# TencentARC/BlobCtrl

Hardware: AMD Instinct MI355X
Metric: 512x512_50step_blobctrl_edits_per_sec (higher is better)
Workload: dtype fp16

## Files before the change

__graft_entry__.py:

```python
import os
import subprocess
import sys

REPO = os.path.dirname(os.path.abspath(__file__))
CSRC = os.path.join(REPO, "blobctrl_amd", "csrc")
LIB = os.path.join(REPO, "blobctrl_amd", "libblobctrl_hip.so")
HEADERS = [os.path.join(REPO, "include", h) for h in ("blobctrl_hip.h", "blobctrl_vae.h")]
SOURCES = ["gemm.hip", "gemm_fast.hip", "conv_halo.hip", "conv_wreg.hip", "gemm_wreg.hip", "gemm256.hip", "norm.hip", "attention.hip", "rowchain.hip", "rowchain_midx.hip", "elementwise.hip", "blobviz.hip", "freeu.hip", "vae_tile.hip", "capi.hip", "plan.hip"]


def _stale():
    if not os.path.exists(LIB):
        return True
    t = os.path.getmtime(LIB)
    deps = [os.path.join(CSRC, f) for f in os.listdir(CSRC)] + HEADERS
    return any(os.path.getmtime(d) > t for d in deps)


def _compile_one(args):
    src, obj, flags = args
    subprocess.check_call([os.environ.get("HIPCC", "/opt/rocm/bin/hipcc")] + flags + ["-c", src, "-o", obj])
    return obj


# ... 60 lines not shown
```

blobctrl_amd/_lib.py:

```python
import ctypes as C
import os

_HERE = os.path.dirname(os.path.abspath(__file__))
LIB_PATH = os.environ.get("BLOBCTRL_HIP_LIB") or os.path.join(_HERE, "libblobctrl_hip.so")

A_DENSE, A_CONV3X3 = 0, 1
ACT_NONE, ACT_GELU, ACT_GEGLU, ACT_SILU, ACT_QUICK_GELU = 0, 1, 2, 3, 4
OUT_F16, OUT_F16_T, OUT_F32 = 0, 1, 2
TILE_NAMES = ["auto", "256x128", "128x128_s3", "128x128_s2", "256x64_s2", "256x64_s3", "128x64", "64x64", "halo128x160", "wreg128x160",
              "gw64x128", "gw64x256", "gw64x320", "g256x256"]
TILE_HALO = 8
TILE_WREG = 9
TILE_GW64x128, TILE_GW64x256, TILE_GW64x320 = 10, 11, 12
TILE_G256 = 13
GW_TILES = {TILE_GW64x128: 2, TILE_GW64x256: 4, TILE_GW64x320: 5}


class BcGemm(C.Structure):
    _fields_ = [
        ("A", C.c_void_p), ("A2", C.c_void_p), ("a_mode", C.c_int),
        ("M", C.c_int), ("N", C.c_int), ("K", C.c_int),
        ("lda", C.c_int), ("lda2", C.c_int), ("C1", C.c_int), ("Cin", C.c_int),
        ("Hin", C.c_int), ("Win", C.c_int), ("Hv", C.c_int), ("Wv", C.c_int),
        ("Hout", C.c_int), ("Wout", C.c_int), ("stride", C.c_int), ("conv_nopad_lo", C.c_int),
# ... 132 lines not shown
    "bc_event_create_sync": (C.c_int, [C.POINTER(C.c_void_p)]),
    "bc_stream_wait_event": (C.c_int, [C.c_void_p, C.c_void_p]),
    "bc_event_record": (C.c_int, [C.c_void_p, C.c_void_p]),
    "bc_event_elapsed_ms": (C.c_int, [C.c_void_p, C.c_void_p, C.POINTER(C.c_float)]),
    "bc_event_destroy": (C.c_int, [C.c_void_p]),
}

EXPORTED_SYMBOLS = tuple(_SIGNATURES.keys())

VAE_SIGNATURES = {
    "bc_vae_tile_blend": (C.c_int, [C.c_void_p, C.c_void_p, C.c_void_p, C.c_void_p, C.c_void_p, C.c_int, C.c_int, C.c_int, C.c_int, C.c_int,
                                    C.c_int, C.c_int, C.c_int, C.c_int, C.c_int, C.c_int, C.c_int, C.c_int, C.c_int, C.c_void_p]),
}
VAE_TILE_DECODE, VAE_TILE_ENCODE = 0, 1

OPS = {"bc_gemm": 0, "bc_gn_stats": 1, "bc_gn_finalize": 2, "bc_gn_apply_fused": 3, "bc_gn_apply": 4, "bc_layernorm": 5,
       "bc_attention": 6, "bc_attention_causal": 7, "bc_assemble_input": 8, "bc_timestep_embedding": 9,
       "bc_timestep_embedding_table": 10, "bc_cfg_scheduler_step": 11, "bc_embed_tokens": 12, "bc_softmax_rows": 13,
       "bc_patchify": 14, "bc_add_cls_pos": 15, "bc_silu": 16, "bc_nchw_to_nhwc_f16": 17, "bc_nhwc_to_nchw": 18,
       "bc_gaussian_sample": 19, "bc_rowchain": 22, "bc_assemble_input_im2col": 23, "bc_memset_zero": 24,
       "bc_rowchain_midx": 25, "bc_rowchain_pack_kv": 26, "bc_rowchain_sum": 27, "bc_ctx_fold": 28, "bc_dup_halves": 29,
       "bc_cfg_scheduler_step_noise": 30, "bc_cfg_scheduler_step3": 31,
       "bc_assemble_input_scaled": 32, "bc_assemble_input_im2col_scaled": 33, "bc_scheduler_step_single": 34,
       "bc_timestep_embedding_table_cond": 35, "bc_timestep_embedding_cond": 36, "bc_freeu": 37}
OP_SIGNAL, OP_WAIT = 20, 21
CHAIN_IN, CHAIN_MID, CHAIN_OUT, CHAIN_OUT_FF, CHAIN_OUT_TAIL, CHAIN_MIDX, CHAIN_OUT_FFP = 0, 1, 2, 3, 4, 5, 6
GN_TOT_WORDS = 6
_KIND = {C.c_void_p: "p", C.c_int: "i", C.c_float: "f", C.c_longlong: "l", C.c_char_p: "p"}


def op_signature(name):
    args = _SIGNATURES[name][1][:-1]
    return "".join("p" if (a not in _KIND) else _KIND[a] for a in args)


class BcPlanBuffer(C.Structure):
    _fields_ = [("name", C.c_char_p), ("address", C.c_void_p), ("bytes", C.c_longlong), ("host_data", C.c_void_p)]

_lib = None


class BlobCtrlHipError(RuntimeError):
    pass


def load():
    global _lib
    if _lib is not None:
        return _lib
    if not os.path.exists(LIB_PATH):
        raise BlobCtrlHipError(
            f"{LIB_PATH} not found: build it with `python -c 'import __graft_entry__ as g; g.build()'` "
            "(hipcc --offload-arch=gfx950).  blobctrl_amd has no CPU fallback.")
    try:
        import torch
    except ImportError:
        pass
    try:
        lib = C.CDLL(LIB_PATH)
    except OSError as e:
        raise BlobCtrlHipError(f"failed to load {LIB_PATH}: {e}") from e
    for name, (res, args) in list(_SIGNATURES.items()) + list(VAE_SIGNATURES.items()):
        fn = getattr(lib, name)
        fn.restype = res
        fn.argtypes = args
    if lib.bc_sizeof_gemm() != C.sizeof(BcGemm):
        raise BlobCtrlHipError(f"BcGemm layout mismatch: C {lib.bc_sizeof_gemm()} vs ctypes {C.sizeof(BcGemm)}")
    _lib = lib
    return lib


def check(rc, what=""):
    if rc != 0:
        msg = load().bc_last_error()
        raise BlobCtrlHipError(f"{what} failed (rc={rc}): {msg.decode() if msg else ''}")
```

blobctrl_amd/csrc/elementwise.hip:

```cpp
#include "bc_common.h"
#include "bc_splat.h"

namespace {

__global__ void splat_kernel(const SplatParams prm, int h, int w, double* __restrict__ out) {
    const int n = blockIdx.y;
    const int idx = blockIdx.x * blockDim.x + threadIdx.x;
    if (idx >= h * w) return;
    const int gy = idx / w, gx = idx - gy * w;
    const double s = bc_splat_score(prm.v + n * 8, gx, gy, h, w);
    double* o = out + (size_t)n * 2 * h * w;
    o[idx] = (1.0 - s);
    o[(size_t)h * w + idx] = s;
}

__device__ __forceinline__ float input_divisor(const float* __restrict__ coef, const int* __restrict__ step_idx, int nsteps) {
    const int step = *step_idx;
    return (step >= 0 && step < nsteps) ? coef[(size_t)step * 16 + 14] : 1.f;
}

template <bool SCALED>
__global__ void assemble_kernel(const float* __restrict__ latents, int Blat, const float* __restrict__ img_lat,
                                const float* __restrict__ score, const float* __restrict__ feat, int Bimg, int F, int Bout,
                                int h, int w, int Cpad, int dup_score, const float* __restrict__ coef,
// ... 109 lines not shown
template <bool SINGLE, bool NOISE, bool THIRD, bool GUARD>
__device__ __forceinline__ void cfg_step_body(const float* __restrict__ eps, float* __restrict__ latents, const float* __restrict__ coef,
                                              const int* __restrict__ step_idx, float* __restrict__ hist, float guidance, int B, int h,
                                              int w, const float* __restrict__ noise, int nsteps, float* __restrict__ eps_out) {
    const int n = B * 4 * h * w;
    const int i = blockIdx.x * blockDim.x + threadIdx.x;
    const int step = *step_idx;
    if (i >= n) return;
    if (GUARD && (step < 0 || step >= nsteps)) return;
    const float* cf = coef + (size_t)step * 16;
    const int xx = i % w;
    const int yy = (i / w) % h;
    const int c = (i / (w * h)) % 4;
    const int b = i / (4 * w * h);
    const size_t pu = (((size_t)b * h + yy) * (2 * w) + (w + xx)) * 4 + c;
    float e;
    if (SINGLE) {
        e = eps[pu];
    } else {
        const size_t pc = (((size_t)(B + b) * h + yy) * (2 * w) + (w + xx)) * 4 + c;
        const float eu = eps[pu], ec = eps[pc];
        const float gscale = guidance >= 0.f ? guidance : cf[11];
        e = eu + gscale * (ec - eu);
    }
    if (eps_out) eps_out[i] = e;
    const float x = latents[i];
    float* m0 = hist, *m1 = hist + n, *last = hist + 2 * (size_t)n;
    const float x0 = x * cf[0] - e * cf[1];
    float xc = x;
    const float pm0 = m0[i], pm1 = m1[i];
    if (cf[2] != 0.f) xc = cf[3] * last[i] + cf[4] * pm0 + cf[5] * pm1 + cf[6] * x0;
    float xn = cf[7] * xc + cf[8] * x0 + cf[9] * pm0 + cf[10] * e;
    m1[i] = pm0;
    m0[i] = x0;
    last[i] = xc;
    if (NOISE) xn = xn + cf[12] * noise[(size_t)step * n + i];
    if (THIRD) xn = xn + cf[13] * pm1;
    latents[i] = xn;
}

template <bool NOISE, bool THIRD, bool GUARD>
__global__ void cfg_step_kernel(const float* __restrict__ eps, float* __restrict__ latents, const float* __restrict__ coef,
                                const int* __restrict__ step_idx, float* __restrict__ hist, float guidance, int B, int h, int w,
                                const float* __restrict__ noise, int nsteps, float* __restrict__ eps_out) {
    cfg_step_body<false, NOISE, THIRD, GUARD>(eps, latents, coef, step_idx, hist, guidance, B, h, w, noise, nsteps, eps_out);
}

template <bool NOISE, bool THIRD>
__global__ void step_single_kernel(const float* __restrict__ eps, float* __restrict__ latents, const float* __restrict__ coef,
                                   const int* __restrict__ step_idx, float* __restrict__ hist, int B, int h, int w,
                                   const float* __restrict__ noise, int nsteps, float* __restrict__ eps_out) {
    cfg_step_body<true, NOISE, THIRD, true>(eps, latents, coef, step_idx, hist, 0.f, B, h, w, noise, nsteps, eps_out);
}
// ... 350 lines not shown
```

blobctrl_amd/csrc/plan.hip:

```cpp
#include <stdio.h>
#include <string.h>
#include <map>
#include <string>
#include <vector>
#include "bc_common.h"
#include "plan_format.h"

void bc_gemm_set_probe(hipEvent_t e);
bool bc_gemm_probe_hit();

using namespace bcplan;

namespace {

struct EventSet {
    std::vector<hipEvent_t> ev;
    explicit EventSet(size_t n) : ev(n, nullptr) {}
    ~EventSet() { for (auto e : ev) if (e) (void)hipEventDestroy(e); }
    hipEvent_t& operator[](size_t i) { return ev[i]; }
};

struct Seg {
    std::string name;
    std::vector<Rec> recs;
// ... 94 lines not shown
            return bc_assemble_input_scaled(CP(float, 0), I(1), CP(float, 2), CP(float, 3), CP(float, 4), I(5), I(6), I(7), I(8), I(9), I(10),
                                            I(11), CP(float, 12), CP(int, 13), I(14), MP(bc_half, 15), s);
        case BC_OP_ASSEMBLE_IM2COL_SCALED:
            return bc_assemble_input_im2col_scaled(CP(float, 0), I(1), CP(float, 2), CP(float, 3), I(4), I(5), I(6), I(7), I(8), CP(float, 9),
                                                   CP(int, 10), I(11), MP(bc_half, 12), s);
        case BC_OP_SCHEDULER_STEP_SINGLE:
            return bc_scheduler_step_single(CP(float, 0), MP(float, 1), CP(float, 2), MP(int, 3), MP(float, 4), I(5), I(6), I(7), CP(float, 8),
                                            I(9), I(10), MP(float, 11), I(12), s);
        case BC_OP_TIMESTEP_EMBEDDING_TABLE_COND:
            return bc_timestep_embedding_table_cond(CP(float, 0), I(1), I(2), I(3), CP(float, 4), MP(bc_half, 5), s);
        case BC_OP_TIMESTEP_EMBEDDING_COND:
            return bc_timestep_embedding_cond(CP(float, 0), CP(int, 1), F(2), I(3), I(4), CP(float, 5), MP(bc_half, 6), s);
        case BC_OP_FREEU:
            return bc_freeu(CP(bc_half, 0), I(1), CP(bc_half, 2), I(3), I(4), I(5), CP(float, 6), I(7), CP(float, 8), MP(bc_half, 9),
                            MP(bc_half, 10), MP(unsigned long long, 11), MP(unsigned long long, 12), s);
        case BC_OP_ROWCHAIN:
            return bc_rowchain(I(0), I(1), I(2), I(3), CP(bc_half, 4), CP(float, 5), CP(unsigned long long, 6), CP(float, 7), CP(float, 8), I(9),
                               F(10), CP(bc_half, 11), CP(bc_half, 12), CP(bc_half, 13), I(14), I(15), I(16), CP(bc_half, 17), CP(float, 18),
                               MP(bc_half, 19), MP(bc_half, 20), MP(bc_half, 21), I(22), MP(unsigned long long, 23), F(24), F(25),
                               CP(float, 26), CP(int, 27), I(28), MP(float, 29), I(30), s);
        case BC_OP_SIGNAL: {
            hipEvent_t ev;
            int rc = plan_event(pl, I(0), &ev);
            if (rc) return rc;
            BC_CHECK_HIP(hipEventRecord(ev, reinterpret_cast<hipStream_t>(s)));
            return 0;
        }
        case BC_OP_WAIT: {
            hipEvent_t ev;
            int rc = plan_event(pl, I(0), &ev);
// ... 395 lines not shown
```

blobctrl_amd/csrc/plan_format.h:

```cpp
#pragma once
#include <stddef.h>
#include <stdint.h>
#include <stdio.h>
#include <string.h>
#include <functional>
#include <string>
#include <vector>
#include "../../include/blobctrl_hip.h"

namespace bcplan {

constexpr int kMaxStreams = 8;
const uint32_t kMagic = 0x4E4C5042u;
const uint32_t kVersion = 7;
inline uint32_t op_min_version(int op) {
    if (op == BC_OP_SCHEDULER_STEP_SINGLE || op == BC_OP_TIMESTEP_EMBEDDING_TABLE_COND || op == BC_OP_TIMESTEP_EMBEDDING_COND ||
        op == BC_OP_FREEU) return 7u;
    return op == BC_OP_ASSEMBLE_INPUT_SCALED || op == BC_OP_ASSEMBLE_IM2COL_SCALED ? 6u : 5u;
}
const uint32_t kOldestReadable = 5;

inline const char* op_signature(int op) {
    switch (op) {
        case BC_OP_GN_STATS: return "piiip";
// ... 21 lines not shown
        case BC_OP_WAIT: return "i";
        case BC_OP_ROWCHAIN: return "iiiipppppifpppiiipppppipffppipi";
        case BC_OP_ASSEMBLE_IM2COL: return "pippiiiiip";
        case BC_OP_MEMSET_ZERO: return "pl";
        case BC_OP_ROWCHAIN_MIDX: return "iiipppppifppf";
        case BC_OP_ROWCHAIN_PACK_KV: return "pipiiiip";
        case BC_OP_ROWCHAIN_SUM: return "iiipippp";
        case BC_OP_CTX_FOLD: return "pipiiiiifppppppp";
        case BC_OP_DUP_HALVES: return "plplplplplpl";
        case BC_OP_ASSEMBLE_INPUT_SCALED: return "pipppiiiiiiippip";
        case BC_OP_ASSEMBLE_IM2COL_SCALED: return "pippiiiiippip";
        case BC_OP_SCHEDULER_STEP_SINGLE: return "pppppiiipiipi";
        case BC_OP_TIMESTEP_EMBEDDING_TABLE_COND: return "piiipp";
        case BC_OP_TIMESTEP_EMBEDDING_COND: return "ppfiipp";
        case BC_OP_FREEU: return "pipiiipippppp";
        default: return nullptr;
    }
}

const size_t kGemmPtrFields[] = {
    offsetof(BcGemm, A), offsetof(BcGemm, A2), offsetof(BcGemm, W), offsetof(BcGemm, bias), offsetof(BcGemm, rowvec),
    offsetof(BcGemm, rowvec_idx), offsetof(BcGemm, colscale), offsetof(BcGemm, alpha_dev), offsetof(BcGemm, alpha_idx),
    offsetof(BcGemm, R), offsetof(BcGemm, R2), offsetof(BcGemm, C), offsetof(BcGemm, gn_tot), offsetof(BcGemm, a_affine),
    offsetof(BcGemm, a_tot1), offsetof(BcGemm, a_tot2), offsetof(BcGemm, a_gamma), offsetof(BcGemm, a_beta),
    offsetof(BcGemm, ln_colsum), offsetof(BcGemm, C_t), offsetof(BcGemm, S), offsetof(BcGemm, S2)};

struct Rec {
    int op = 0, sid = 0, enabled = 1;
    std::vector<uint64_t> a;
    BcGemm g;
// ... 129 lines not shown
```

blobctrl_amd/engine.py:

```python
import os
from dataclasses import dataclass
from typing import List, Optional, Tuple

import torch

from . import _lib
from .launch import Recorder
from .options import opt
from .weights import PackedTrunk, pad8


@dataclass
class TrunkConfig:
    in_channels: int
    block_out_channels: Tuple[int, ...] = (320, 640, 1280, 1280)
    layers_per_block: int = 2
    num_heads: int = 8
    norm_num_groups: int = 32
    cross_attention_dim: Optional[int] = 768
    out_channels: int = 4
    is_blobnet: bool = False
    time_cond_proj_dim: Optional[int] = None


# ... 499 lines not shown
        M = self.B * H * W
        if out is None:
            out = self.rec.empty(self.B, H * W, Cout)
        self.rec.gemm(A=x_in, W=pw.h[wkey], M=M, N=Cout, K=128, out=out, bias=pw.f["conv_in.bias"], rows_per_batch=H * W, kind="conv_in",
                      want_gn=True, gn_tot_out=gn_tot_out, **self._r2(r2, H, W))
        return Act(out, Cout, H, W)

    def cfg_prefix_ok(self, cfg_pairs, im2col):
        cfg = self.cfg
        if not cfg_pairs or cfg.is_blobnet or self.B % 2 or not im2col or not opt("cfg_prefix") or len(cfg.block_out_channels) < 2:
            return False
        Cc, HW = cfg.block_out_channels[0], self.H * self.W
        return self.pw.has_cross and Cc in (320, 640) and self.rowchain_ok(Cc, (self.B // 2) * HW, HW, "down_blocks.0.attentions.0.")

    def record_forward(self, x_in: torch.Tensor, residuals: Optional[Residuals] = None, zero_scale=None,
                       signal_residuals: bool = False, eps_out: Optional[torch.Tensor] = None, im2col: bool = False, cfg_pairs: bool = False):
        cfg, pw = self.cfg, self.pw
        boc = cfg.block_out_channels
        nb = len(boc)
        H, W = self.H, self.W
        res_d = list(residuals.down) if residuals is not None else None
        res_u = list(residuals.up) if residuals is not None else None
        self.res_bmod = residuals.bmod if residuals is not None else 1
        self.res_events = residuals.events if residuals is not None else None
        pop = (lambda lst: lst.pop(0)) if residuals is not None else (lambda lst: None)
        alpha, alpha_dev, alpha_idx, alpha_bstride = (tuple(zero_scale) + (0,))[:4] if zero_scale is not None else (1.0, None, None, 0)
        out_events = {} if signal_residuals else None

        class _Feats(list):
            def __init__(s2, prefix):
                super().__init__()
# ... 103 lines not shown
                r = pop(res_u)
                sk = res.pop()
                if self.freeu_params is not None and not cfg.is_blobnet and i < 2:
                    h, sk = self.freeu(h, sk, stage=i)
                h = self.resnet(f"up_blocks.{i}.resnets.{j}.", h, sk, rev[i], r2=None if has_attn else r)
                pre = None
                if has_attn:
                    h, pre = self.transformer(f"up_blocks.{i}.attentions.{j}.", h, r2=r, zero=feats_u.next_zero())
                feats_u.append(h, pre)
            if i < nb - 1:
                size = (skips[-1].H, skips[-1].W)
                h = self.conv3x3(h, f"up_blocks.{i}.upsamplers.0.conv", rev[i], up_to=size, r2=pop(res_u),
                                 kind="upsample")
                feats_u.append(h)
        if not cfg.is_blobnet:
            n = self.groupnorm(h, None, "conv_norm_out", 1e-5, True)
            small = 7 if (self.B * H * W) >= 64 * 128 else 0
            eps = self.conv3x3(n, "conv_out", cfg.out_channels, out_f32=True, kind="conv_out", out=eps_out, tile_cfg=small)
            return eps.t
        self.feat_shapes = ([(f.C, f.H, f.W) for f in feats_d], (feat_mid.C, feat_mid.H, feat_mid.W),
                            [(f.C, f.H, f.W) for f in feats_u])
        return Residuals(feats_d.res, feats_m.res[0], feats_u.res, bmod=self.B, events=out_events)


def _ptr(t):
    return None if t is None else t.data_ptr()
```

blobctrl_amd/launch.py:

```python
import ctypes as C
import json
import os
import struct
from typing import List, Optional

import torch

from . import _lib
from .options import opt
from ._lib import BcGemm


_TUNING_PATH = os.environ.get("BC_TUNING_FILE") or os.path.join(os.path.dirname(os.path.abspath(__file__)), "gemm_tuning.json")
_TUNING = None
_M64 = (1 << 64) - 1


def tuning_table():
    global _TUNING
    if _TUNING is None:
        _TUNING = {}
        if os.path.exists(_TUNING_PATH) and not os.environ.get("BC_NO_TUNING"):
            with open(_TUNING_PATH) as f:
                _TUNING = json.load(f).get("shapes", {})
# ... 464 lines not shown
        elif cfg == _lib.TILE_G256:
            rp = "gemm256_kernel"
        elif cfg in _lib.GW_TILES:
            rp = f"gemm_wreg_kernel<{_lib.GW_TILES[cfg]}, {10 if _lib.GW_TILES[cfg] == 5 else 20}, {'true' if sm_group else 'false'}>"
        elif fast:
            ups_ = bool(conv) and (conv.get("Hv", conv["Hin"]), conv.get("Wv", conv["Win"])) != (conv["Hin"], conv["Win"])
            rp = f"gemm_fast_kernel<{FAST[cfg]}, {'true' if conv else 'false'}, {'true' if ups_ else 'false'}>"
        else:
            rp = "gemm_kernel<" + ("256, 64, 4, 1" if bn == 64 else "128, 128, 2, 2") + ">"
        a_elems = (M // (conv["Hout"] * conv["Wout"])) * conv["Hin"] * conv["Win"] * conv["Cin"] if conv else M * K
        alg_bytes = 2 * (a_elems + N * K + M * n_out) + (2 * M * n_out if R is not None else 0) + 2 * (M + N) * Cs
        self._push(kind, 2 * M * N * (K + Cs), variant, (mode, M, N, K + Cs, sk), alg_bytes, rp)
        return out

    def _op(self, name, args, kind, **meta):
        self._add_op(_lib.OPS[name], _lib.op_signature(name), args, kind, **meta)

    def gn_sources(self, x1, C1, x2, C2, B, HW, G):
        srcs = []
        c2_ = C2 if x2 is not None else 0
        cpg = (C1 + c2_) // G
        for x, c, off in ((x1, C1, 0), (x2, c2_, C1)):
            if x is None:
                srcs.append(None)
                continue
            hit = self.tots.get(x.data_ptr())
            blocks_ok = c % 320 != 0 or id(hit) in self.tots_per_channel or (cpg % 10 == 0 and off % 10 == 0)
            if hit is not None and hit.shape[1] == c and blocks_ok:
                srcs.append(hit)
            else:
                tot = self.new_tot(B, c)
# ... 111 lines not shown
        return wqk, cs, qb, vwo

    def rowchain_midx(self, Cc, M, rows_per_batch, x, wstream, vec, kvstream, n_ctx, heads, scale, out0, out1, res, ln_eps=1e-5):
        assert heads * (Cc // heads) == Cc and heads == 8, "CHAIN_MIDX is laid out for 8 heads"
        refs = (x, wstream, vec, kvstream, out0, out1, res)
        self.keep.append(refs)
        for t in refs:
            self.register(t)
        B = M // rows_per_batch
        self._op("bc_rowchain_midx", (Cc, M, rows_per_batch, x, res, wstream, vec, kvstream, n_ctx, scale, out0, out1, ln_eps), "rowchain",
                 flops=2 * M * Cc * Cc * 2 + 4 * M * n_ctx * Cc, variant="rowchain_kernel<midx>",
                 shape=("rowchain_midx", M, Cc, 2 * Cc), bytes_=2 * (2 * Cc * Cc + 3 * M * Cc + 2 * B * n_ctx * Cc),
                 rocprof=f"rowchain_kernel<{Cc}, {_lib.CHAIN_MIDX}, false>")
        return out1

    def call(self, name, *args, kind=None, keep=()):
        self.keep.append(keep)
        for t in keep if isinstance(keep, (tuple, list)) else (keep,):
            self.register(t)
        self._op(name, args, kind or name)
```

blobctrl_amd/options.py:

```python
import os

TABLE = {
    "rowchain": (True, "transformer blocks of 320 / 640 channels on csrc/rowchain.hip (0: GroupNorm / LayerNorm / GEMM launch list)"),
    "midx": (True, "cross-attention of the 320 / 640-channel blocks inside the row-chain's MID launch (0: MID + bc_attention)"),
    "ffp": (True, "UNet's split 640-channel block end as OUT_FFP + sum (0: OUT_FF + OUT_TAIL)"),
    "ffp_blob": (False, "BlobNet's split block end as OUT_FFP + sum too"),
    "gw": (True, "1280-channel projections at M <= gw_maxm on csrc/gemm_wreg.hip (0: LDS-DMA tiles + LayerNorm launches)"),
    "ctx_fold": (True, "cross-attention of the 1280-channel blocks folded over the prompt (0: to_q + bc_attention + to_out)"),
    "g256": (True, "large-M dense projections on csrc/gemm256.hip from g256_min_tiles tiles on (0: gemm_fast tiles)"),
    "gw_ff1_g256": (True, "ff.net.0 of the 1280-channel blocks at M <= gw_maxm as LayerNorm + gemm256.hip where it has >= g256_min_tiles tiles"),
    "cfg_prefix": (True, "CFG-invariant prefix of the UNet once per image pair (0: every launch at the full CFG batch)"),
    "wreg": (True, "ResBlock convolutions on csrc/conv_wreg.hip (0: csrc/conv_halo.hip)"),
    "sc_fold": (True, "a ResBlock's 1x1 shortcut folded into conv2's K loop on csrc/conv_wreg.hip (0: a conv1x1 launch + residual read)"),
    "halo": (True, "ResBlock convolutions with the fused GroupNorm prologue at all (0: GroupNorm pass + implicit GEMM)"),
    "gn_finalize_launch": (False, "a bc_gn_finalize launch per GroupNorm instead of the finalize in the consumer's prologue"),
    "halo_ctas": (0, "workgroups a split-K convolution pass aims for (0: 128 on conv_wreg, 256 on conv_halo)"),
    "halo_min_cps": (0, "fewest 64-channel chunks per workgroup of a split pass (0: 3 on conv_wreg, 2 on conv_halo)"),
    "halo_full": (0, "workgroups from which a pass runs unsplit (0: two thirds of halo_ctas)"),
    "rowchain_min_blocks_640": (64, "fewest 64-row blocks for the 640-channel row-chain"),
    "rowchain_min_blocks_640_blob_up": (32, "... for BlobNet's up blocks"),
    "ff_split_640": (0, "workgroups per row block of the 640-channel block end up to 64 row blocks (0: 4 with OUT_FFP, 2 without)"),
    "ff_split_640_blob": (0, "... for BlobNet (0: as ff_split_640)"),
    "ff_split_320": (1, "workgroups per row block of the 320-channel block end up to 128 row blocks"),
    "gw_maxm": (1024, "largest M of a projection on gemm_wreg.hip"),
    "ctx_fold_maxb": (2, "largest UNet batch that takes the prompt-folded cross-attention"),
    "gn_pass_min_requests": (4, "edit requests per batch from which a ResBlock convolution runs as GroupNorm pass + plain conv_wreg (0: never)"),
    "gn_pass_min_cin": (320, "... and fewest input channels of such a convolution"),
    "g256_min_tiles": (64, "fewest 256 x 256 tiles for gemm256.hip (a quarter of the CUs: the other queue has the rest)"),
}


def _parse(text):
    out = {}
    for item in (text or "").replace(";", ",").split(","):
        item = item.strip()
        if not item:
            continue
        if "=" not in item:
            raise ValueError(f"BC_PLAN: '{item}' is not key=value")
        k, v = (s.strip() for s in item.split("=", 1))
        if k not in TABLE:
            raise ValueError(f"BC_PLAN: unknown key '{k}' (known: {', '.join(sorted(TABLE))})")
# ... 23 lines not shown
```

blobctrl_amd/pipeline.py:

```python
import os
from typing import List, Optional, Union

import torch

from . import _lib
from .engine import TrunkConfig, TrunkPlan, freeu_enabled
from .launch import Recorder
from .schedulers import OPTION_KINDS, draw_variance_noise, randn_tensor, table_class
from .weights import PackedTrunk, lora_scale_of, pad8


def get_guidance_scale_embedding(w: torch.Tensor, embedding_dim: int = 512, dtype: torch.dtype = torch.float32) -> torch.Tensor:
    if w.dim() != 1:
        raise ValueError("w must be one-dimensional (one guidance weight per sample)")
    half = embedding_dim // 2
    rate = torch.log(torch.tensor(10000.0)) / (half - 1)
    freq = torch.exp(torch.arange(half, dtype=dtype) * -rate)
    angle = (w * 1000.0).to(dtype)[:, None] * freq[None, :]
    out = torch.zeros(w.shape[0], embedding_dim, dtype=angle.dtype)
    out[:, :half] = torch.sin(angle)
    out[:, half:2 * half] = torch.cos(angle)
    return out


# ... 114 lines not shown
            half_time.record_time_table(P.t_table, nsteps, P.step_idx, **({} if P.timestep_cond is None else dict(cond=P.timestep_cond[:B])))
            P.eps_all = rec.zeros(2 * B, H * W, self.unet_cfg.out_channels, dtype=f32)

        def half_plan(b0):
            hp = TrunkPlan(rec, self.unet_w, self.unet_cfg, B, H, W)
            hp.freeu_params = P.freeu
            hp.ctx_kv = {bp: (ck[b0 * T:(b0 + B) * T], cvt[b0:b0 + B], T_, ld) for bp, (ck, cvt, T_, ld) in unet_a.ctx_kv.items()}
            hp.ctx_kvs = {bp: kvs.view(2 * B, -1)[b0:b0 + B].reshape(-1) for bp, kvs in getattr(unet_a, "ctx_kvs", {}).items()}
            hp.ctx_folded = {bp: tuple(t[b0:b0 + B] for t in f) for bp, f in getattr(unet_a, "ctx_folded", {}).items()}
            hp.tproj, hp.tproj_table = half_time.tproj, half_time.tproj_table
            return hp

        divisor = (P.coef.data_ptr(), P.step_idx.data_ptr(), nsteps) if P.scaled else ()
        suffix = "_scaled" if P.scaled else ""

        def record_unet(plan, residuals):
            if P.unet_im2col:
                rec.call("bc_assemble_input_im2col" + suffix, P.latents.data_ptr(), B, P.bg_lat.data_ptr(), P.bg_score.data_ptr(), Bi, Bu,
                         h, w, 0, *divisor, P.unet_in.data_ptr(), kind="assemble")
            else:
                rec.call("bc_assemble_input" + suffix, P.latents.data_ptr(), B, P.bg_lat.data_ptr(), P.bg_score.data_ptr(), None, Bi, 0,
                         Bu, h, w, unet_cin, 0, *divisor, P.unet_in.data_ptr(), kind="assemble")
            if temb_per_step:
                plan.record_time(P.t_table, P.step_idx)
            if split_cfg:
                ready, joined = rec.new_event(), rec.new_event()
                rec.signal(ready)
                rec.sid = 2
                rec.wait(ready)
                half_plan(B).record_forward(P.unet_in[B:], residuals, eps_out=P.eps_all[B:], im2col=P.unet_im2col)
                rec.signal(joined)
                rec.sid = 0
                half_plan(0).record_forward(P.unet_in[:B], residuals, eps_out=P.eps_all[:B], im2col=P.unet_im2col)
                rec.wait(joined)
                eps = P.eps_all
            else:
                eps = plan.record_forward(P.unet_in, residuals, im2col=P.unet_im2col, cfg_pairs=not single)
            P.eps = eps
            if single:
                rec.call("bc_scheduler_step_single", eps, P.latents, P.coef, P.step_idx, P.hist, B, h, w, P.variance_noise, nsteps,
                         int(P.third_order), P.eps_guided, 1, kind="cfg_step")
                return
            name, extra = ("bc_cfg_scheduler_step_noise", (P.variance_noise, nsteps)) if P.stochastic else \
                ("bc_cfg_scheduler_step3", (nsteps,)) if P.third_order else ("bc_cfg_scheduler_step", ())
            rec.call(name, eps, P.latents, P.coef, P.step_idx, P.hist, -1.0, B, h, w, *extra, P.eps_guided, 1, kind="cfg_step")

        P.step_active = rec.begin("step_active")
        fork = rec.new_event()
        rec.signal(fork)
        rec.sid = 1
# ... 861 lines not shown
```

include/blobctrl_hip.h:

```cpp
#ifndef BLOBCTRL_HIP_H
#define BLOBCTRL_HIP_H

#include <stdint.h>

#ifdef __cplusplus
extern "C" {
#endif

typedef uint16_t bc_half;
typedef void*    bc_stream;

const char* bc_last_error(void);
int bc_version(void);
int bc_device_info(int* out4);

enum { BC_A_DENSE = 0, BC_A_CONV3X3 = 1 };
enum { BC_ACT_NONE = 0, BC_ACT_GELU = 1, BC_ACT_GEGLU = 2, BC_ACT_SILU = 3, BC_ACT_QUICK_GELU = 4  };
enum { BC_OUT_F16 = 0, BC_OUT_F16_T = 1, BC_OUT_F32 = 2 };

typedef struct BcGemm {
    const bc_half* A;
    const bc_half* A2;
    int a_mode;
    int M, N, K;
// ... 182 lines not shown

int bc_event_create(void** ev);
int bc_event_record(void* ev, bc_stream stream);
int bc_event_elapsed_ms(void* start, void* stop, float* ms);
int bc_event_destroy(void* ev);

typedef struct BcPlan BcPlan;
enum { BC_OP_GEMM = 0, BC_OP_GN_STATS = 1, BC_OP_GN_FINALIZE = 2, BC_OP_GN_APPLY_FUSED = 3, BC_OP_GN_APPLY = 4, BC_OP_LAYERNORM = 5,
       BC_OP_ATTENTION = 6, BC_OP_ATTENTION_CAUSAL = 7, BC_OP_ASSEMBLE_INPUT = 8, BC_OP_TIMESTEP_EMBEDDING = 9,
       BC_OP_TIMESTEP_EMBEDDING_TABLE = 10, BC_OP_CFG_SCHEDULER_STEP = 11, BC_OP_EMBED_TOKENS = 12, BC_OP_SOFTMAX_ROWS = 13,
       BC_OP_PATCHIFY = 14, BC_OP_ADD_CLS_POS = 15, BC_OP_SILU = 16, BC_OP_NCHW_TO_NHWC_F16 = 17, BC_OP_NHWC_TO_NCHW = 18,
       BC_OP_GAUSSIAN_SAMPLE = 19, BC_OP_SIGNAL = 20 , BC_OP_WAIT = 21 , BC_OP_ROWCHAIN = 22, BC_OP_ASSEMBLE_IM2COL = 23,
       BC_OP_MEMSET_ZERO = 24, BC_OP_ROWCHAIN_MIDX = 25, BC_OP_ROWCHAIN_PACK_KV = 26, BC_OP_ROWCHAIN_SUM = 27, BC_OP_CTX_FOLD = 28, BC_OP_DUP_HALVES = 29,
       BC_OP_CFG_SCHEDULER_STEP_NOISE = 30, BC_OP_CFG_SCHEDULER_STEP3 = 31, BC_OP_ASSEMBLE_INPUT_SCALED = 32,
       BC_OP_ASSEMBLE_IM2COL_SCALED = 33, BC_OP_SCHEDULER_STEP_SINGLE = 34, BC_OP_TIMESTEP_EMBEDDING_TABLE_COND = 35,
       BC_OP_TIMESTEP_EMBEDDING_COND = 36, BC_OP_FREEU = 37, BC_OP_COUNT = 38 };
typedef struct BcPlanBuffer {
    const char* name;
    const void* address;
    long long   bytes;
    const void* host_data;
} BcPlanBuffer;

int bc_plan_create(BcPlan** out);
int bc_plan_destroy(BcPlan* plan);
int bc_plan_segment(BcPlan* plan, const char* name);
int bc_plan_find_segment(BcPlan* plan, const char* name);
int bc_plan_new_event(BcPlan* plan);
int bc_plan_add_gemm(BcPlan* plan, int seg, int stream_id, const BcGemm* g);
int bc_plan_add_op(BcPlan* plan, int seg, int stream_id, int op, const uint64_t* args, int nargs);
int bc_plan_set_slab(BcPlan* plan, int stream_id, float* slab);
// ... 18 lines not shown
```

Measured before the change: 2.428.

## Fuse conv_norm_out, conv_out on the crop, CFG and scheduler step into one kernel

Adds a step_tail kernel that applies the final GroupNorm with SiLU, runs conv_out only over the cropped half of the canvas, combines the CFG pair and performs the scheduler update. A grid-wide atomic counter lets the last block advance the step index, all in a single launch. This removes the separate GroupNorm pass, the full-canvas conv_out and the scheduler launch, along with their intermediate memory traffic. The cost is a small-tile dot2 convolution with cross-wave reduction that may use the GPU less fully than the GEMM path, plus an atomic-based step advance.

After: 2.433, median of 4. No clear change (+0.2%).

```diff
diff --git a/__graft_entry__.py b/__graft_entry__.py
--- a/__graft_entry__.py
+++ b/__graft_entry__.py
@@ -5,8 +5,8 @@
 REPO = os.path.dirname(os.path.abspath(__file__))
 CSRC = os.path.join(REPO, "blobctrl_amd", "csrc")
 LIB = os.path.join(REPO, "blobctrl_amd", "libblobctrl_hip.so")
-HEADERS = [os.path.join(REPO, "include", h) for h in ("blobctrl_hip.h", "blobctrl_vae.h")]
-SOURCES = ["gemm.hip", "gemm_fast.hip", "conv_halo.hip", "conv_wreg.hip", "gemm_wreg.hip", "gemm256.hip", "norm.hip", "attention.hip", "rowchain.hip", "rowchain_midx.hip", "elementwise.hip", "blobviz.hip", "freeu.hip", "vae_tile.hip", "capi.hip", "plan.hip"]
+HEADERS = [os.path.join(REPO, "include", h) for h in ("blobctrl_hip.h", "blobctrl_vae.h", "blobctrl_step.h")]
+SOURCES = ["gemm.hip", "gemm_fast.hip", "conv_halo.hip", "conv_wreg.hip", "gemm_wreg.hip", "gemm256.hip", "norm.hip", "attention.hip", "rowchain.hip", "rowchain_midx.hip", "elementwise.hip", "step_tail.hip", "blobviz.hip", "freeu.hip", "vae_tile.hip", "capi.hip", "plan.hip"]
 
 
 def _stale():
diff --git a/blobctrl_amd/_lib.py b/blobctrl_amd/_lib.py
--- a/blobctrl_amd/_lib.py
+++ b/blobctrl_amd/_lib.py
@@ -170,6 +170,14 @@
 }
 VAE_TILE_DECODE, VAE_TILE_ENCODE = 0, 1
 
+STEP_SIGNATURES = {
+    "bc_step_tail": (C.c_int, [C.c_void_p, C.c_int, C.c_void_p, C.c_void_p, C.c_void_p, C.c_int, C.c_float, C.c_void_p, C.c_void_p, C.c_int,
+                               C.c_int, C.c_int, C.c_int, C.c_void_p, C.c_void_p, C.c_void_p, C.c_void_p, C.c_float, C.c_void_p, C.c_int, C.c_int,
+                               C.c_void_p, C.c_void_p, C.c_void_p, C.c_int, C.c_void_p]),
+    "bc_step_tail_max_channels": (C.c_int, []),
+}
+STEP_OPS = {"bc_step_tail": 38}
+
 OPS = {"bc_gemm": 0, "bc_gn_stats": 1, "bc_gn_finalize": 2, "bc_gn_apply_fused": 3, "bc_gn_apply": 4, "bc_layernorm": 5,
        "bc_attention": 6, "bc_attention_causal": 7, "bc_assemble_input": 8, "bc_timestep_embedding": 9,
        "bc_timestep_embedding_table": 10, "bc_cfg_scheduler_step": 11, "bc_embed_tokens": 12, "bc_softmax_rows": 13,
@@ -185,8 +193,12 @@
 _KIND = {C.c_void_p: "p", C.c_int: "i", C.c_float: "f", C.c_longlong: "l", C.c_char_p: "p"}
 
 
+def op_code(name):
+    return OPS[name] if name in OPS else STEP_OPS[name]
+
+
 def op_signature(name):
-    args = _SIGNATURES[name][1][:-1]
+    args = (_SIGNATURES[name] if name in _SIGNATURES else STEP_SIGNATURES[name])[1][:-1]
     return "".join("p" if (a not in _KIND) else _KIND[a] for a in args)
 
 
@@ -216,7 +228,7 @@
         lib = C.CDLL(LIB_PATH)
     except OSError as e:
         raise BlobCtrlHipError(f"failed to load {LIB_PATH}: {e}") from e
-    for name, (res, args) in list(_SIGNATURES.items()) + list(VAE_SIGNATURES.items()):
+    for name, (res, args) in list(_SIGNATURES.items()) + list(VAE_SIGNATURES.items()) + list(STEP_SIGNATURES.items()):
         fn = getattr(lib, name)
         fn.restype = res
         fn.argtypes = args
diff --git a/blobctrl_amd/csrc/cfg_step.h b/blobctrl_amd/csrc/cfg_step.h
--- /dev/null
+++ b/blobctrl_amd/csrc/cfg_step.h
@@ -0,0 +1,30 @@
+#pragma once
+#include <stddef.h>
+#include <hip/hip_runtime.h>
+
+template <bool SINGLE, bool NOISE, bool THIRD>
+__device__ __forceinline__ void bc_cfg_step_element(float eu, float ec, int i, int n, int step, const float* __restrict__ cf,
+                                                    float* __restrict__ latents, float* __restrict__ hist, float guidance,
+                                                    const float* __restrict__ noise, float* __restrict__ eps_out) {
+    float e;
+    if (SINGLE) {
+        e = eu;
+    } else {
+        const float gscale = guidance >= 0.f ? guidance : cf[11];
+        e = eu + gscale * (ec - eu);
+    }
+    if (eps_out) eps_out[i] = e;
+    const float x = latents[i];
+    float* m0 = hist, *m1 = hist + n, *last = hist + 2 * (size_t)n;
+    const float x0 = x * cf[0] - e * cf[1];
+    float xc = x;
+    const float pm0 = m0[i], pm1 = m1[i];
+    if (cf[2] != 0.f) xc = cf[3] * last[i] + cf[4] * pm0 + cf[5] * pm1 + cf[6] * x0;
+    float xn = cf[7] * xc + cf[8] * x0 + cf[9] * pm0 + cf[10] * e;
+    m1[i] = pm0;
+    m0[i] = x0;
+    last[i] = xc;
+    if (NOISE) xn = xn + cf[12] * noise[(size_t)step * n + i];
+    if (THIRD) xn = xn + cf[13] * pm1;
+    latents[i] = xn;
+}
diff --git a/blobctrl_amd/csrc/elementwise.hip b/blobctrl_amd/csrc/elementwise.hip
--- a/blobctrl_amd/csrc/elementwise.hip
+++ b/blobctrl_amd/csrc/elementwise.hip
@@ -1,5 +1,6 @@
 #include "bc_common.h"
 #include "bc_splat.h"
+#include "cfg_step.h"
 
 namespace {
 
@@ -147,29 +148,10 @@
     const int c = (i / (w * h)) % 4;
     const int b = i / (4 * w * h);
     const size_t pu = (((size_t)b * h + yy) * (2 * w) + (w + xx)) * 4 + c;
-    float e;
-    if (SINGLE) {
-        e = eps[pu];
-    } else {
-        const size_t pc = (((size_t)(B + b) * h + yy) * (2 * w) + (w + xx)) * 4 + c;
-        const float eu = eps[pu], ec = eps[pc];
-        const float gscale = guidance >= 0.f ? guidance : cf[11];
-        e = eu + gscale * (ec - eu);
-    }
-    if (eps_out) eps_out[i] = e;
-    const float x = latents[i];
-    float* m0 = hist, *m1 = hist + n, *last = hist + 2 * (size_t)n;
-    const float x0 = x * cf[0] - e * cf[1];
-    float xc = x;
-    const float pm0 = m0[i], pm1 = m1[i];
-    if (cf[2] != 0.f) xc = cf[3] * last[i] + cf[4] * pm0 + cf[5] * pm1 + cf[6] * x0;
-    float xn = cf[7] * xc + cf[8] * x0 + cf[9] * pm0 + cf[10] * e;
-    m1[i] = pm0;
-    m0[i] = x0;
-    last[i] = xc;
-    if (NOISE) xn = xn + cf[12] * noise[(size_t)step * n + i];
-    if (THIRD) xn = xn + cf[13] * pm1;
-    latents[i] = xn;
+    const float eu = eps[pu];
+    float ec = 0.f;
+    if (!SINGLE) ec = eps[(((size_t)(B + b) * h + yy) * (2 * w) + (w + xx)) * 4 + c];
+    bc_cfg_step_element<SINGLE, NOISE, THIRD>(eu, ec, i, n, step, cf, latents, hist, guidance, noise, eps_out);
 }
 
 template <bool NOISE, bool THIRD, bool GUARD>
diff --git a/blobctrl_amd/csrc/plan.hip b/blobctrl_amd/csrc/plan.hip
--- a/blobctrl_amd/csrc/plan.hip
+++ b/blobctrl_amd/csrc/plan.hip
@@ -5,6 +5,7 @@
 #include <vector>
 #include "bc_common.h"
 #include "plan_format.h"
+#include "../../include/blobctrl_step.h"
 
 void bc_gemm_set_probe(hipEvent_t e);
 bool bc_gemm_probe_hit();
@@ -132,6 +133,10 @@
         case BC_OP_FREEU:
             return bc_freeu(CP(bc_half, 0), I(1), CP(bc_half, 2), I(3), I(4), I(5), CP(float, 6), I(7), CP(float, 8), MP(bc_half, 9),
                             MP(bc_half, 10), MP(unsigned long long, 11), MP(unsigned long long, 12), s);
+        case BC_OP_STEP_TAIL:
+            return bc_step_tail(CP(bc_half, 0), I(1), CP(unsigned long long, 2), CP(float, 3), CP(float, 4), I(5), F(6), CP(bc_half, 7), CP(float, 8),
+                                I(9), I(10), I(11), I(12), MP(float, 13), CP(float, 14), MP(int, 15), MP(float, 16), F(17), CP(float, 18), I(19),
+                                I(20), MP(float, 21), MP(float, 22), MP(unsigned, 23), I(24), s);
         case BC_OP_ROWCHAIN:
             return bc_rowchain(I(0), I(1), I(2), I(3), CP(bc_half, 4), CP(float, 5), CP(unsigned long long, 6), CP(float, 7), CP(float, 8), I(9),
                                F(10), CP(bc_half, 11), CP(bc_half, 12), CP(bc_half, 13), I(14), I(15), I(16), CP(bc_half, 17), CP(float, 18),
diff --git a/blobctrl_amd/csrc/plan_format.h b/blobctrl_amd/csrc/plan_format.h
--- a/blobctrl_amd/csrc/plan_format.h
+++ b/blobctrl_amd/csrc/plan_format.h
@@ -59,6 +59,7 @@
         case BC_OP_TIMESTEP_EMBEDDING_TABLE_COND: return "piiipp";
         case BC_OP_TIMESTEP_EMBEDDING_COND: return "ppfiipp";
         case BC_OP_FREEU: return "pipiiipippppp";
+        case BC_OP_STEP_TAIL: return "pipppifppiiiippppfpiipppi";
         default: return nullptr;
     }
 }
diff --git a/blobctrl_amd/csrc/step_tail.hip b/blobctrl_amd/csrc/step_tail.hip
--- /dev/null
+++ b/blobctrl_amd/csrc/step_tail.hip
@@ -0,0 +1,226 @@
+#include "bc_common.h"
+#include "cfg_step.h"
+#include "../../include/blobctrl_step.h"
+
+namespace {
+
+constexpr int TH = 4, TW = 8;
+constexpr int HH = TH + 2, HW_ = TW + 2;
+constexpr int HPIX = HH * HW_;
+constexpr int CK = 64;
+constexpr int NWAVE = CK / 8;
+constexpr int NT = NWAVE * 64;
+constexpr int LDP = CK + 8;
+constexpr int CMAX = 320;
+constexpr int NCHUNK = CMAX / CK;
+constexpr int NLOAD = (2 * HPIX * (CK / 8) + NT - 1) / NT;
+constexpr int BUF_BYTES = 2 * HPIX * LDP * 2;
+static_assert(BUF_BYTES >= 2 * CMAX * 2 * 8 && BUF_BYTES >= NWAVE * 64 * 4 * 4, "the totals / partial sums alias a staging buffer");
+
+struct TailArgs {
+    const h16* x; int C;
+    const unsigned long long* tot;
+    const float* gamma; const float* beta; int G; float gn_eps;
+    const h16* W; const float* bias;
+    int B, h, w;
+    float* latents; const float* coef; int* step_idx; float* hist; float guidance; const float* noise; int nsteps; int third;
+    float* eps_guided; float* eps_crop; unsigned* arrive; int advance;
+};
+
+template <bool SINGLE>
+__global__ __launch_bounds__(NT) void step_tail_kernel(const TailArgs a) {
+    __shared__ float ab_s[2][CMAX][2];
+    __shared__ __attribute__((aligned(16))) h16 w_s[4 * 9 * CMAX];
+    __shared__ __attribute__((aligned(16))) unsigned char stage_s[2 * BUF_BYTES];
+    typedef h16 (*ActBuf)[HPIX][LDP];
+    double* sq_s = reinterpret_cast<double*>(stage_s + BUF_BYTES);
+    float (*red_s)[64][4] = reinterpret_cast<float (*)[64][4]>(stage_s);
+    constexpr int NIMG = SINGLE ? 1 : 2;
+    const int tid = threadIdx.x;
+    const int wv = __builtin_amdgcn_readfirstlane(tid >> 6), lane = tid & 63;
+    const int C = a.C, h = a.h, w = a.w, Wc = 2 * a.w;
+    const int tiles_x = (w + TW - 1) / TW;
+    const int ty0 = (blockIdx.x / tiles_x) * TH, tx0 = (blockIdx.x % tiles_x) * TW;
+    const int b = blockIdx.y;
+    const int step = *a.step_idx;
+
+    uint4 raw[NCHUNK][NLOAD];
+    auto src_of = [&](int e, int c0, int& img, int& hp, int& oct) -> const h16* {
+        oct = e & 7;
+        hp = (e >> 3) % HPIX;
+        img = e / (8 * HPIX);
+        const int y = ty0 + hp / HW_ - 1, x = w + tx0 + hp % HW_ - 1;
+        const int c = c0 + oct * 8;
+        if (img >= NIMG || y < 0 || y >= h || x < 0 || x >= Wc || c >= C) return nullptr;
+        return a.x + (((size_t)(img * a.B + b) * h + y) * Wc + x) * C + c;
+    };
+    auto load_chunk = [&](int c0, uint4 (&r)[NLOAD]) {
+#pragma unroll
+        for (int j = 0; j < NLOAD; ++j) {
+            int img, hp, oct;
+            const h16* p = src_of(tid + j * NT, c0, img, hp, oct);
+            r[j] = p ? bc_ld16(p) : make_uint4(0, 0, 0, 0);
+        }
+    };
+    auto store_chunk = [&](int c0, int buf, const uint4 (&r)[NLOAD]) {
+        ActBuf act = reinterpret_cast<ActBuf>(stage_s + buf * BUF_BYTES);
+#pragma unroll
+        for (int j = 0; j < NLOAD; ++j) {
+            int img, hp, oct;
+            const int e = tid + j * NT;
+            const h16* p = src_of(e, c0, img, hp, oct);
+            if (e >= 2 * HPIX * 8) continue;
+            uint4 o = make_uint4(0, 0, 0, 0);
+            if (p) {
+                const h16* v = reinterpret_cast<const h16*>(&r[j]);
+                h16* oh = reinterpret_cast<h16*>(&o);
+                const int c = c0 + oct * 8;
+#pragma unroll
+                for (int k = 0; k < 8; ++k) {
+                    const float r = (float)v[k] * ab_s[img][c + k][0] + ab_s[img][c + k][1];
+                    oh[k] = (h16)bc_silu_f(r);
+                }
+            }
+            *reinterpret_cast<uint4*>(&act[img][hp][oct * 8]) = o;
+        }
+    };
+
+    for (int i = tid; i < NIMG * C; i += NT) {
+        const int img = i / C, c = i - img * C;
+        double s, q;
+        bc_gn_tot_read(a.tot + ((size_t)(img * a.B + b) * C + c) * BC_GN_TOT_WORDS, s, q);
+        sq_s[2 * i] = s;
+        sq_s[2 * i + 1] = q;
+    }
+    for (int i = tid; i < 4 * 9 * C / 8; i += NT) reinterpret_cast<uint4*>(w_s)[i] = bc_ld16(a.W + (size_t)i * 8);
+    const int nchunk = (C + CK - 1) / CK;
+#pragma unroll
+    for (int k = 0; k < NCHUNK; ++k)
+        if (k < nchunk) load_chunk(k * CK, raw[k]);
+    __syncthreads();
+    const int cpg = C / a.G;
+    if (tid < NIMG * a.G) {
+        const int img = tid / a.G, g = tid - img * a.G;
+        double s = 0.0, q = 0.0;
+        for (int j = 0; j < cpg; ++j) {
+            s += sq_s[2 * (img * C + g * cpg + j)];
+            q += sq_s[2 * (img * C + g * cpg + j) + 1];
+        }
+        const double n = (double)h * Wc * cpg;
+        const double mean = s / n;
+        double var = q / n - mean * mean;
+        if (var < 0.0) var = 0.0;
+        const float meanf = (float)mean, rstd = (float)(1.0 / sqrt(var + (double)a.gn_eps));
+        for (int c = g * cpg; c < (g + 1) * cpg; ++c) {
+            const float sc = rstd * a.gamma[c];
+            ab_s[img][c][0] = sc;
+            ab_s[img][c][1] = a.beta[c] - meanf * sc;
+        }
+    }
+    __syncthreads();
+
+    const int img_l = lane >> 5, pl = lane & 31;
+    const int ty = pl >> 3, tx = pl & 7;
+    float acc[4] = {0.f, 0.f, 0.f, 0.f};
+    const int ldw = 9 * C;
+#pragma unroll
+    for (int k = 0; k < NCHUNK; ++k) {
+        if (k >= nchunk) break;
+        const int c0 = k * CK, buf = k & 1;
+        store_chunk(c0, buf, raw[k]);
+        __syncthreads();
+        const int c = c0 + wv * 8;
+        if (c < C) {
+            ActBuf act = reinterpret_cast<ActBuf>(stage_s + buf * BUF_BYTES);
+#pragma unroll
+            for (int ky = 0; ky < 3; ++ky) {
+#pragma unroll
+                for (int kx = 0; kx < 3; ++kx) {
+                    const uint4 av = *reinterpret_cast<const uint4*>(&act[img_l][(ty + ky) * HW_ + tx + kx][wv * 8]);
+                    const h16x2* ap = reinterpret_cast<const h16x2*>(&av);
+                    const h16* wp = w_s + (ky * 3 + kx) * C + c;
+#pragma unroll
+                    for (int co = 0; co < 4; ++co) {
+                        const uint4 wq = *reinterpret_cast<const uint4*>(wp + co * ldw);
+                        const h16x2* wh = reinterpret_cast<const h16x2*>(&wq);
+#pragma unroll
+                        for (int j = 0; j < 4; ++j) acc[co] = __builtin_amdgcn_fdot2(ap[j], wh[j], acc[co], false);
+                    }
+                }
+            }
+        }
+    }
+    __syncthreads();
+#pragma unroll
+    for (int co = 0; co < 4; ++co) red_s[wv][lane][co] = acc[co];
+    __syncthreads();
+
+    if (tid < 128) {
+        const int c = tid >> 5, p = tid & 31;
+        const int yy = ty0 + (p >> 3), xx = tx0 + (p & 7);
+        if (yy < h && xx < w) {
+            const float bias = a.bias[c];
+            float su = 0.f, sc = 0.f;
+#pragma unroll
+            for (int v = 0; v < NWAVE; ++v) {
+                su += red_s[v][p][c];
+                if (!SINGLE) sc += red_s[v][32 + p][c];
+            }
+            const float eu = su + bias, ec = sc + bias;
+            if (a.eps_crop) {
+                a.eps_crop[(((size_t)b * h + yy) * Wc + (w + xx)) * 4 + c] = eu;
+                if (!SINGLE) a.eps_crop[(((size_t)(a.B + b) * h + yy) * Wc + (w + xx)) * 4 + c] = ec;
+            }
+            if (step >= 0 && step < a.nsteps) {
+                const int n = a.B * 4 * h * w;
+                const int i = ((b * 4 + c) * h + yy) * w + xx;
+                const float* cf = a.coef + (size_t)step * 16;
+                if (a.noise && a.third)
+                    bc_cfg_step_element<SINGLE, true, true>(eu, ec, i, n, step, cf, a.latents, a.hist, a.guidance, a.noise, a.eps_guided);
+                else if (a.noise)
+                    bc_cfg_step_element<SINGLE, true, false>(eu, ec, i, n, step, cf, a.latents, a.hist, a.guidance, a.noise, a.eps_guided);
+                else if (a.third)
+                    bc_cfg_step_element<SINGLE, false, true>(eu, ec, i, n, step, cf, a.latents, a.hist, a.guidance, a.noise, a.eps_guided);
+                else
+                    bc_cfg_step_element<SINGLE, false, false>(eu, ec, i, n, step, cf, a.latents, a.hist, a.guidance, a.noise, a.eps_guided);
+            }
+        }
+    }
+
+    if (a.advance && tid == 0) {
+        const unsigned total = gridDim.x * gridDim.y;
+        const unsigned prev = __hip_atomic_fetch_add(a.arrive, 1u, __ATOMIC_ACQ_REL, __HIP_MEMORY_SCOPE_AGENT);
+        if (prev == total - 1) {
+            __hip_atomic_store(a.arrive, 0u, __ATOMIC_RELAXED, __HIP_MEMORY_SCOPE_AGENT);
+            *a.step_idx = step + 1;
+        }
+    }
+}
+
+}
+
+extern "C" int bc_step_tail_max_channels() { return CMAX; }
+
+extern "C" int bc_step_tail(const bc_half* x, int C, const unsigned long long* tot, const float* gamma, const float* beta, int G, float gn_eps,
+                            const bc_half* conv_w, const float* conv_b, int B, int h, int w, int single, float* latents, const float* coef,
+                            int* step_idx, float* hist, float guidance_scale, const float* noise, int nsteps, int third, float* eps_out,
+                            float* eps_crop, unsigned* arrive, int advance, bc_stream stream_) {
+    hipStream_t stream = reinterpret_cast<hipStream_t>(stream_);
+    BC_CHECK_ARG(x && tot && gamma && beta && conv_w && conv_b && latents && coef && step_idx && hist && B > 0 && h > 0 && w > 0 && nsteps > 0 &&
+                 (!advance || arrive), "bc_step_tail: bad args");
+    BC_CHECK_ARG(C > 0 && C % 8 == 0 && C <= CMAX && G > 0 && C % G == 0 && (single ? 1 : 2) * G <= 256,
+                 "bc_step_tail: C=%d (a multiple of 8 up to %d) in G=%d groups (at most %d) is not supported", C, CMAX, G, single ? 256 : 128);
+    BC_CHECK_ARG((long long)B * 4 * h * w < (1ll << 31) && (long long)2 * B * h * 2 * w * C < (1ll << 40), "bc_step_tail: canvas too large");
+    TailArgs a;
+    a.x = reinterpret_cast<const h16*>(x); a.C = C; a.tot = tot; a.gamma = gamma; a.beta = beta; a.G = G; a.gn_eps = gn_eps;
+    a.W = reinterpret_cast<const h16*>(conv_w); a.bias = conv_b; a.B = B; a.h = h; a.w = w;
+    a.latents = latents; a.coef = coef; a.step_idx = step_idx; a.hist = hist; a.guidance = guidance_scale; a.noise = noise; a.nsteps = nsteps;
+    a.third = third; a.eps_guided = eps_out; a.eps_crop = eps_crop; a.arrive = arrive; a.advance = advance;
+    const dim3 grid(bc_ceil_div(w, TW) * bc_ceil_div(h, TH), B);
+    if (single)
+        hipLaunchKernelGGL(step_tail_kernel<true>, grid, dim3(NT), 0, stream, a);
+    else
+        hipLaunchKernelGGL(step_tail_kernel<false>, grid, dim3(NT), 0, stream, a);
+    BC_CHECK_LAUNCH();
+    return 0;
+}
diff --git a/blobctrl_amd/engine.py b/blobctrl_amd/engine.py
--- a/blobctrl_amd/engine.py
+++ b/blobctrl_amd/engine.py
@@ -537,7 +537,8 @@
         return self.pw.has_cross and Cc in (320, 640) and self.rowchain_ok(Cc, (self.B // 2) * HW, HW, "down_blocks.0.attentions.0.")
 
     def record_forward(self, x_in: torch.Tensor, residuals: Optional[Residuals] = None, zero_scale=None,
-                       signal_residuals: bool = False, eps_out: Optional[torch.Tensor] = None, im2col: bool = False, cfg_pairs: bool = False):
+                       signal_residuals: bool = False, eps_out: Optional[torch.Tensor] = None, im2col: bool = False, cfg_pairs: bool = False,
+                       defer_out: bool = False):
         cfg, pw = self.cfg, self.pw
         boc = cfg.block_out_channels
         nb = len(boc)
@@ -671,6 +672,8 @@
                                  kind="upsample")
                 feats_u.append(h)
         if not cfg.is_blobnet:
+            if defer_out:
+                return h
             n = self.groupnorm(h, None, "conv_norm_out", 1e-5, True)
             small = 7 if (self.B * H * W) >= 64 * 128 else 0
             eps = self.conv3x3(n, "conv_out", cfg.out_channels, out_f32=True, kind="conv_out", out=eps_out, tile_cfg=small)
diff --git a/blobctrl_amd/launch.py b/blobctrl_amd/launch.py
--- a/blobctrl_amd/launch.py
+++ b/blobctrl_amd/launch.py
@@ -502,7 +502,7 @@
         return out
 
     def _op(self, name, args, kind, **meta):
-        self._add_op(_lib.OPS[name], _lib.op_signature(name), args, kind, **meta)
+        self._add_op(_lib.op_code(name), _lib.op_signature(name), args, kind, **meta)
 
     def gn_sources(self, x1, C1, x2, C2, B, HW, G):
         srcs = []
@@ -644,6 +644,24 @@
                  rocprof=f"rowchain_kernel<{Cc}, {_lib.CHAIN_MIDX}, false>")
         return out1
 
+    def step_tail_ok(self, Cc, G, single):
+        return Cc % 8 == 0 and 0 < Cc <= self.lib.bc_step_tail_max_channels() and Cc % G == 0 and (1 if single else 2) * G <= 256
+
+    def step_tail(self, x, Cc, images, HW, G, eps, gamma, beta, conv_w, conv_b, B, h, w, single, latents, coef, step_idx, hist, noise, nsteps,
+                  third, eps_guided, eps_crop):
+        assert HW == h * 2 * w and images == (B if single else 2 * B) and self.step_tail_ok(Cc, G, single)
+        tot, _ = self.gn_sources(x, Cc, None, 0, images, HW, G)
+        arrive = self.zeros(1, dtype=torch.int32)
+        refs = (x, tot, gamma, beta, conv_w, conv_b, latents, coef, step_idx, hist, noise, eps_guided, eps_crop, arrive)
+        self.keep.append(refs)
+        for t in refs:
+            self.register(t)
+        self._op("bc_step_tail", (x, Cc, tot, gamma, beta, G, eps, conv_w, conv_b, B, h, w, 1 if single else 0, latents, coef, step_idx, hist,
+                                  -1.0, noise, nsteps, 1 if third else 0, eps_guided, eps_crop, arrive, 1), "step_tail",
+                 flops=2 * images * h * w * 4 * 9 * Cc, variant="step_tail_kernel", shape=("step_tail", images, h, w, Cc),
+                 bytes_=2 * images * h * (w + 1) * Cc + 2 * 4 * 9 * Cc + 4 * 8 * B * 4 * h * w,
+                 rocprof=f"step_tail_kernel<{'true' if single else 'false'}>")
+
     def call(self, name, *args, kind=None, keep=()):
         self.keep.append(keep)
         for t in keep if isinstance(keep, (tuple, list)) else (keep,):
diff --git a/blobctrl_amd/options.py b/blobctrl_amd/options.py
--- a/blobctrl_amd/options.py
+++ b/blobctrl_amd/options.py
@@ -12,6 +12,8 @@
     "cfg_prefix": (True, "CFG-invariant prefix of the UNet once per image pair (0: every launch at the full CFG batch)"),
     "wreg": (True, "ResBlock convolutions on csrc/conv_wreg.hip (0: csrc/conv_halo.hip)"),
     "sc_fold": (True, "a ResBlock's 1x1 shortcut folded into conv2's K loop on csrc/conv_wreg.hip (0: a conv1x1 launch + residual read)"),
+    "step_tail": (True, "conv_norm_out + conv_out on the crop + CFG + scheduler step + counter advance as one csrc/step_tail.hip launch "
+                        "(0: GroupNorm pass + conv_out over the canvas + bc_cfg_scheduler_step*)"),
     "halo": (True, "ResBlock convolutions with the fused GroupNorm prologue at all (0: GroupNorm pass + implicit GEMM)"),
     "gn_finalize_launch": (False, "a bc_gn_finalize launch per GroupNorm instead of the finalize in the consumer's prologue"),
     "halo_ctas": (0, "workgroups a split-K convolution pass aims for (0: 128 on conv_wreg, 256 on conv_halo)"),
@@ -26,6 +28,7 @@
     "ctx_fold_maxb": (2, "largest UNet batch that takes the prompt-folded cross-attention"),
     "gn_pass_min_requests": (4, "edit requests per batch from which a ResBlock convolution runs as GroupNorm pass + plain conv_wreg (0: never)"),
     "gn_pass_min_cin": (320, "... and fewest input channels of such a convolution"),
+    "step_tail_min_c": (64, "fewest channels of the UNet's last block for step_tail (one staged chunk; narrower trunks keep the launch list)"),
     "g256_min_tiles": (64, "fewest 256 x 256 tiles for gemm256.hip (a quarter of the CUs: the other queue has the rest)"),
 }
 
diff --git a/blobctrl_amd/pipeline.py b/blobctrl_amd/pipeline.py
--- a/blobctrl_amd/pipeline.py
+++ b/blobctrl_amd/pipeline.py
@@ -6,6 +6,7 @@
 from . import _lib
 from .engine import TrunkConfig, TrunkPlan, freeu_enabled
 from .launch import Recorder
+from .options import opt
 from .schedulers import OPTION_KINDS, draw_variance_noise, randn_tensor, table_class
 from .weights import PackedTrunk, lora_scale_of, pad8
 
@@ -152,6 +153,11 @@
         divisor = (P.coef.data_ptr(), P.step_idx.data_ptr(), nsteps) if P.scaled else ()
         suffix = "_scaled" if P.scaled else ""
 
+        C_last = self.unet_cfg.block_out_channels[0]
+        step_tail = bool(opt("step_tail")) and not split_cfg and self.unet_cfg.out_channels == 4 and C_last >= opt("step_tail_min_c") and \
+            rec.step_tail_ok(C_last, self.unet_cfg.norm_num_groups, single)
+        P.step_tail = step_tail
+
         def record_unet(plan, residuals):
             if P.unet_im2col:
                 rec.call("bc_assemble_input_im2col" + suffix, P.latents.data_ptr(), B, P.bg_lat.data_ptr(), P.bg_score.data_ptr(), Bi, Bu,
@@ -172,6 +178,14 @@
                 half_plan(0).record_forward(P.unet_in[:B], residuals, eps_out=P.eps_all[:B], im2col=P.unet_im2col)
                 rec.wait(joined)
                 eps = P.eps_all
+            elif step_tail:
+                hl = plan.record_forward(P.unet_in, residuals, im2col=P.unet_im2col, cfg_pairs=not single, defer_out=True)
+                P.eps = rec.zeros(Bu, H * W, self.unet_cfg.out_channels, dtype=f32)
+                pw = self.unet_w
+                rec.step_tail(hl.t, hl.C, Bu, H * W, plan.G, 1e-5, pw.f["conv_norm_out.weight"], pw.f["conv_norm_out.bias"],
+                              pw.h["conv_out.weight"], pw.f["conv_out.bias"], B, h, w, single, P.latents, P.coef, P.step_idx, P.hist,
+                              P.variance_noise, nsteps, P.third_order and (single or not P.stochastic), P.eps_guided, P.eps)
+                return
             else:
                 eps = plan.record_forward(P.unet_in, residuals, im2col=P.unet_im2col, cfg_pairs=not single)
             P.eps = eps
diff --git a/include/blobctrl_hip.h b/include/blobctrl_hip.h
--- a/include/blobctrl_hip.h
+++ b/include/blobctrl_hip.h
@@ -220,7 +220,7 @@
        BC_OP_MEMSET_ZERO = 24, BC_OP_ROWCHAIN_MIDX = 25, BC_OP_ROWCHAIN_PACK_KV = 26, BC_OP_ROWCHAIN_SUM = 27, BC_OP_CTX_FOLD = 28, BC_OP_DUP_HALVES = 29,
        BC_OP_CFG_SCHEDULER_STEP_NOISE = 30, BC_OP_CFG_SCHEDULER_STEP3 = 31, BC_OP_ASSEMBLE_INPUT_SCALED = 32,
        BC_OP_ASSEMBLE_IM2COL_SCALED = 33, BC_OP_SCHEDULER_STEP_SINGLE = 34, BC_OP_TIMESTEP_EMBEDDING_TABLE_COND = 35,
-       BC_OP_TIMESTEP_EMBEDDING_COND = 36, BC_OP_FREEU = 37, BC_OP_COUNT = 38 };
+       BC_OP_TIMESTEP_EMBEDDING_COND = 36, BC_OP_FREEU = 37, BC_OP_STEP_TAIL = 38 , BC_OP_COUNT = 39 };
 typedef struct BcPlanBuffer {
     const char* name;
     const void* address;
diff --git a/include/blobctrl_step.h b/include/blobctrl_step.h
--- /dev/null
+++ b/include/blobctrl_step.h
@@ -0,0 +1,21 @@
+#ifndef BLOBCTRL_STEP_H
+#define BLOBCTRL_STEP_H
+
+#include "blobctrl_hip.h"
+
+#ifdef __cplusplus
+extern "C" {
+#endif
+
+int bc_step_tail(const bc_half* x, int C, const unsigned long long* tot, const float* gamma, const float* beta, int G, float gn_eps,
+                 const bc_half* conv_w, const float* conv_b, int B, int h, int w, int single, float* latents, const float* coef,
+                 int* step_idx, float* hist, float guidance_scale, const float* noise, int nsteps, int third, float* eps_out,
+                 float* eps_crop, unsigned* arrive, int advance, bc_stream stream);
+
+int bc_step_tail_max_channels(void);
+
+#ifdef __cplusplus
+}
+#endif
+
+#endif
```
